# juanmc2005/diart

Measured on NVIDIA H100. Metric: audio-seconds/sec (real-time factor) at 5s/0.5s step, batch 256, higher is better.
Workload: dtype f32

## Files before the change

### diart_b200/_lib.py

```python
from __future__ import annotations

import ctypes as C
import os
from typing import Dict, Optional

import numpy as np
import torch

_HERE = os.path.dirname(os.path.abspath(__file__))
LIB_PATH = os.path.join(_HERE, "libdiartb200.so")

_lib: Optional[C.CDLL] = None


class DgTensor(C.Structure):
    _fields_ = [("name", C.c_char_p), ("data", C.c_void_p), ("numel", C.c_int64)]


_P = C.c_void_p
SIGNATURES = {
    "dg_last_error": (C.c_char_p, []),
    "dg_version": (C.c_int, []),
    "dg_launch_count": (C.c_int64, []),
    "dg_profile_enable": (C.c_int, [C.c_int]),
    "dg_profile_report": (C.c_int, [C.c_char_p, C.c_int]),
    "dg_selftest_gemm_tc": (C.c_int, [C.c_int, C.c_int, C.c_int, C.c_int, C.c_int, C.c_int, C.POINTER(C.c_float),
                                      C.POINTER(C.c_float)]),
    "dg_selftest_gemm_tc_grid": (C.c_int, [C.c_int, C.c_int, C.c_int, C.c_int, C.c_int, C.c_int, C.POINTER(C.c_int)]),
    "dg_selftest_gemm_tc_bounds": (C.c_int, [C.c_int, C.c_int, C.c_int, C.c_int, C.POINTER(C.c_int), C.POINTER(C.c_int),
                                             C.POINTER(C.c_int)]),
    "dg_selftest_wgmma_row_shift": (C.c_int, [C.c_int, C.POINTER(C.c_uint)]),
    "dg_selftest_gemm_tc_halo": (C.c_int, [C.c_int, C.c_int, C.c_int, C.c_int, C.c_int, C.c_int, C.POINTER(C.c_int),
                                           C.POINTER(C.c_int)]),
    "dg_selftest_split_f16_host": (C.c_int, [_P, C.c_longlong, _P, _P]),
    "dg_seg_create": (C.c_int, [C.POINTER(DgTensor), C.c_int, C.c_int, C.POINTER(_P)]),
    "dg_seg_dims": (C.c_int, [_P, C.c_int, C.POINTER(C.c_int), C.POINTER(C.c_int)]),
    "dg_seg_set_powerset": (C.c_int, [_P, C.c_int, C.c_int]),
    "dg_seg_forward": (C.c_int, [_P, _P, C.c_int, C.c_int, _P, _P]),
    "dg_seg_destroy": (C.c_int, [_P]),
    "dg_emb_create": (C.c_int, [C.POINTER(DgTensor), C.c_int, C.c_int, C.c_int, C.POINTER(_P)]),
    "dg_emb_dims": (C.c_int, [_P, C.c_int, C.POINTER(C.c_int), C.POINTER(C.c_int)]),
    "dg_emb_forward": (C.c_int, [_P, _P, _P, C.c_int, C.c_int, C.c_int, C.c_int, C.c_int, C.c_float, _P, _P]),
    "dg_emb_forward_rows": (C.c_int, [_P, _P, _P, C.c_int, C.c_int, C.c_int, _P, _P]),
    "dg_emb_destroy": (C.c_int, [_P]),
    "dg_emb_debug_trunk": (C.c_int, [_P, _P, C.c_int, C.c_int, C.c_int, _P, C.c_int64, _P]),
    "dg_seg_debug_stage": (C.c_int, [_P, _P, C.c_int, C.c_int, C.c_int, C.c_int, _P, C.c_int64, _P]),
    "dg_emb_debug_stage": (C.c_int, [_P, _P, _P, C.c_int, C.c_int, C.c_int, C.c_int, C.c_int, C.c_int, _P, C.c_int64, _P]),
    "dg_selftest_sinc_filters_host": (C.c_int, [_P, _P, _P]),
    "dg_selftest_fbank_tables_host": (C.c_int, [_P, _P]),
    "dg_osp": (C.c_int, [_P, C.c_int, C.c_int, C.c_int, C.c_float, C.c_float, C.c_int, _P, _P]),
    "dg_normalize_embeddings": (C.c_int, [_P, C.c_int, C.c_int, C.c_float, _P, _P]),
    "dg_cluster_create": (C.c_int, [C.c_int, C.c_int, C.c_double, C.c_double, C.c_double, C.c_int, C.POINTER(_P)]),
    "dg_cluster_set_metric": (C.c_int, [_P, C.c_int]),
    "dg_cluster_step": (C.c_int, [_P, _P, _P, C.c_int, C.c_int, C.c_int, _P, _P, _P]),
    "dg_cluster_reset": (C.c_int, [_P]),
    "dg_cluster_get_state": (C.c_int, [_P, _P, _P, C.POINTER(C.c_int)]),
    "dg_cluster_set_state": (C.c_int, [_P, _P, _P, C.c_int]),
    "dg_cluster_destroy": (C.c_int, [_P]),
    "dg_cluster_record_len": (C.c_int, [_P]),
    "dg_cluster_export_delta": (C.c_int, [_P, _P, _P]),
    "dg_cluster_merge": (C.c_int, [_P, _P, C.c_int, C.c_int, _P, C.c_int, _P]),
    "dg_pipeline_identity_export": (C.c_int, [_P, _P, _P]),
    "dg_pipeline_identity_merge": (C.c_int, [_P, _P, C.c_int, C.c_int, _P]),
    "dg_pipeline_create": (C.c_int, [_P, _P, _P, C.c_float, C.c_float, C.c_int, C.POINTER(_P)]),
    "dg_pipeline_set_hop": (C.c_int, [_P, C.c_int]),
    "dg_pipeline_step": (C.c_int, [_P, _P, C.c_int, C.c_int, _P, _P, _P, _P, _P]),
# ... 152 lines not shown
```

### diart_b200/csrc/api.cu

```cuda
#include <math.h>
#include <stdlib.h>
#include <string.h>

#include <map>
#include <sstream>
#include <vector>

#include "host.cuh"

namespace dg {

static thread_local std::string g_err;
std::atomic<long long> g_launches{0};
thread_local int g_sm_limit = 0;
void set_error(const std::string& msg) { g_err = msg; }

struct ProfRec {
  std::string name;
  cudaEvent_t a, b;
};
static bool g_prof = false;
static std::vector<ProfRec> g_recs;
static const bool g_trace = getenv("DG_TRACE_LAUNCHES") && getenv("DG_TRACE_LAUNCHES")[0] == '1';
ProfScope::ProfScope(const char* name_, cudaStream_t st_) : on(g_prof), st(st_), a(nullptr), b(nullptr), name(name_) {
// ... 337 lines not shown
    t.pool3_tile_rows = tile_rows;
  }
  if ((rc = set_weights(t, dW))) return rc;
  *halo = gemm_tc_halo(t) ? 1 : 0;
  TcGemm ref = t;
  ref.tap_boxes = 1;
  if (folded) {
    ref.Cin = Kf;
    ref.KW = 1;
    if ((rc = set_weights(ref, dWf))) return rc;
  }
  std::vector<unsigned char> first, cur;
  *equal = 1;
  for (int run = 0; run < 3; run++) {
    DG_CUDA(cudaMemset(dF.p, 0, f32_bytes + 4));
    DG_CUDA(cudaMemset(dOh.p, 0, plane_bytes + 4));
    DG_CUDA(cudaMemset(dOl.p, 0, plane_bytes + 4));
    DG_CUDA(cudaMemset(dPart.p, 0, part_bytes + 4));
    {
      SmLimit cap(run == 1 ? 3 : 0);
      if ((rc = launch_gemm_tc(run == 2 ? ref : t, nullptr))) return rc;
    }
    DG_CUDA(cudaDeviceSynchronize());
    cur.resize(f32_bytes + 2 * plane_bytes + part_bytes);
    DG_CUDA(cudaMemcpy(cur.data(), dF.p, f32_bytes, cudaMemcpyDeviceToHost));
    DG_CUDA(cudaMemcpy(cur.data() + f32_bytes, dOh.p, plane_bytes, cudaMemcpyDeviceToHost));
    DG_CUDA(cudaMemcpy(cur.data() + f32_bytes + plane_bytes, dOl.p, plane_bytes, cudaMemcpyDeviceToHost));
    DG_CUDA(cudaMemcpy(cur.data() + f32_bytes + 2 * plane_bytes, dPart.p, part_bytes, cudaMemcpyDeviceToHost));
    if (run == 0)
      first.swap(cur);
    else if (cur != first)
      *equal = 0;
  }
  return DG_OK;
}

extern "C" int dg_selftest_gemm_tc_bounds(int M, int Cin, int N, int epi, int* outside_unchanged, int* equal, int* refused) {
  const bool planes = epi == 1;
  if (M < 1 || Cin < 64 || Cin % 64 || N < 1 || N % (planes ? 32 : 4) || epi < 0 || epi > 2 || !outside_unchanged || !equal ||
      !refused) {
    set_error("dg_selftest_gemm_tc_bounds: bad arguments");
    return DG_EINVAL;
  }
  const int npad = N <= 64 && epi == 0 ? 64 : (N + 127) / 128 * 128, esize = planes ? 2 : 4;
  const int ldc = N + 40;
  const long long rows = (long long)M + 130;
  uint32_t seed = 4242u;
  auto rnd = [&]() {
    seed = seed * 1664525u + 1013904223u;
    return ((seed >> 8) & 0xFFFF) / 65536.f - 0.5f;
  };
  std::vector<float> A((size_t)M * Cin), Wnk((size_t)N * Cin), bias(N), bsc(N), bsh(N);
  for (auto& v : A) v = 2.f * rnd();
  for (auto& v : Wnk) v = 0.25f * rnd();
  for (int n = 0; n < N; n++) {
    bias[n] = rnd();
    bsc[n] = 1.f + rnd();
    bsh[n] = rnd();
  }
  const size_t dense_bytes = (size_t)M * N * esize, wide_bytes = (size_t)rows * ldc * esize + 16;
  DevBuf dA, dAh, dAl, dB, dS, dH, dD0, dD1, dW0, dW1;
  WeightPlanes dW;
  if (upload(dA, A) || upload(dB, bias) || upload(dS, bsc) || upload(dH, bsh) || upload_split(dW, Wnk, N, npad, Cin) ||
      dAh.ensure((size_t)M * Cin * 2) || dAl.ensure((size_t)M * Cin * 2) || dD0.ensure(dense_bytes) ||
      dD1.ensure(dense_bytes) || dW0.ensure(wide_bytes) || dW1.ensure(wide_bytes))
    return DG_ECUDA;
// ... 49 lines not shown
```

### diart_b200/csrc/dg_common.cuh

```cuda
#pragma once
#include <cuda_runtime.h>
#include <stdint.h>
#include <stdio.h>

#include <atomic>
#include <string>
#include <vector>

namespace dg {

void set_error(const std::string& msg);
extern std::atomic<long long> g_launches;
extern thread_local int g_sm_limit;
inline int usable_sms() {
  int dev = 0, sms = 132;
  cudaGetDevice(&dev);
  cudaDeviceGetAttribute(&sms, cudaDevAttrMultiProcessorCount, dev);
  return (g_sm_limit > 0 && g_sm_limit < sms) ? g_sm_limit : sms;
}

#define DG_CUDA(expr)                                                                   \
  do {                                                                                  \
    cudaError_t _e = (expr);                                                            \
    if (_e != cudaSuccess) {                                                            \
// ... 92 lines not shown
  int lda, Cin, KW, dil;
  long long Mtot, M;
  const void* W_hi;
  const void* W_lo;
  float w_scale;
  int Npad, N;
  const float* bias;
  const float* bn_scale;
  const float* bn_shift;
  float* out_f32;
  void* out_hi;
  void* out_lo;
  int ldc;
  int epi;
  const char* tag;
  const int* tap_off;
  int Wp, Hp, Wop, Hop, stride2, relu;
  const void* res_hi;
  const void* res_lo;
  const float* pool_w;
  float* pool_part;
  int pool_item_rows, pool_K;
  int pool_T;
  int pool3_T, pool3_tile_rows;
  int tap_boxes;
};
inline int gemm_tc_pool3_tile_rows(int item_rows) {
  for (int t = 126; t >= 96; t -= 3)
    if (item_rows % t == 0) return t;
  return 0;
}
int launch_gemm_tc(const TcGemm& g, cudaStream_t st);
bool gemm_tc_halo(const TcGemm& g);
int selftest_wgmma_row_shift(int base_offset_mode, unsigned* ok_shifts);
int launch_split_ex(const float* x, long long rows_out, int C, int ld_in, int ld_out, int pool, int item_rows,
                    const float* sc, const float* sh, void* hi, void* lo, cudaStream_t st, const int* skip_flag = nullptr);
void split_weights_host(const float* w, int N, int Npad, int K, uint16_t* hi, uint16_t* lo, float scale = 1.f);
float weight_plane_scale(const float* w, size_t n);
uint16_t host_f32_to_h16(float f);
float host_h16_to_f32(uint16_t h);
int sinc_tc_rows_per_item(const Geom& g);
size_t sinc_tc_plane_elems(int B, const Geom& g);
void sinc_tc_pack_filters(const float* filt, uint16_t* planes );
void sinc_tc_affine_consts(const float* filt, float beta, float* cf);
int launch_sinc_prep(const float* wav, const float* mean, const float* rstd, int B, const Geom& g, void* planes_hi,
                     void* planes_lo, cudaStream_t st, const int* skip_flag = nullptr);
int launch_sinc0_tc(float gamma, const float* cf_dev, const void* w_planes, int B, const Geom& g, const void* planes_hi,
                    const void* planes_lo, float* p0, cudaStream_t st, const int* skip_flag = nullptr);
struct SincStreamGeom {
  int Ls;
  int P;
  int rows;
  size_t plane;
};
SincStreamGeom sinc_stream_geom(int B, const Geom& g, int hop);
int launch_overlap_check(const float* wav, int B, int S, int hop, int* flag, cudaStream_t st);
int launch_stream_prep(const float* wav, const float* rstd, int B, const Geom& g, int hop, void* planes_hi, void* planes_lo,
                       int* flag, cudaStream_t st);
int launch_sinc0_tc_stream(const void* w_planes, int B, const Geom& g, int hop, const void* planes_hi, const void* planes_lo,
                           float* craw, const int* flag, cudaStream_t st);
size_t sinc_pool_part_floats(int B, const Geom& g, int hop);
int launch_sinc_pool_fused(const float* craw, const float* mean, const float* rstd, const float* cf, const float* hsum, float gamma,
                           int B, const Geom& g, int hop, const float* g0, const float* b0, float* part, float* sc, float* sh,
                           void* planes_hi, void* planes_lo, const int* flag, cudaStream_t st);
size_t lstm_tc_plane_elems();
int lstm_tc_rows(int B);
// ... 161 lines not shown
```

### diart_b200/csrc/gemm_tc.cu

```cuda
#include <cuda.h>
#include <cuda_bf16.h>
#include <math.h>
#include <stdlib.h>
#include <string.h>

#include <algorithm>
#include <map>
#include <mutex>
#include <string>
#include <utility>
#include <vector>

#include "dg_common.cuh"
#include "tc_ptx.cuh"

namespace dg {

constexpr int TC_BM = 128, TC_BK = 32, TC_THREADS = 384;
constexpr int TC_SMEM_MAX = 227 * 1024;

struct TcArgs {
  long long M;
  int N;
  int m_tiles, n_tiles;
// ... 26 lines not shown

__host__ __device__ constexpr bool tc_pooling(int epi) { return epi == TC_POOL || epi == TC_MAXPOOL3; }
__host__ __device__ constexpr bool tc_box_store(int epi) { return epi == TC_BIAS_F32 || epi == TC_LEAKY_BN_SPLIT || epi == TC_LEAKY_BN_F32; }

template <int BN>
struct TcSmem {
  static constexpr int A_BYTES = TC_BM * TC_BK * 2;
  static constexpr int W_BYTES = BN * TC_BK * 2;
  static constexpr int STAGE_BYTES = 2 * A_BYTES + 2 * W_BYTES;
  static constexpr int W_STAGE_BYTES = 2 * W_BYTES;
  static constexpr int NSTAGE = BN == 128 ? 4 : 6;
  static constexpr int NSTAGE_HALO = BN == 128 ? 5 : 6;
  __host__ static int halo_bytes(int cin, int rows) { return (2 * ((cin + 31) / 32) * rows * 64 + 1023) / 1024 * 1024; }
  __host__ static int halo_op_bytes(int cin, int rows) { return 2 * halo_bytes(cin, rows) + NSTAGE_HALO * W_STAGE_BYTES; }
  static constexpr int BAR_BYTES = 256;
  static constexpr int PARAM_FLOATS = 3 * BN;
  static constexpr int CHUNK_W = 64;
  static constexpr int CHUNK_FLOATS = CHUNK_W / 32 * TC_BM * 33;
  __host__ __device__ static constexpr int extra_floats(int epi) { return epi == TC_POOL ? 128 * 4 + 4 * 2 * 8 * 32 : (epi == TC_MAXPOOL3 ? 4 * 2 * 2 * 32 : 0); }
  __host__ __device__ static constexpr int consumer_floats(int epi) { return PARAM_FLOATS + (tc_pooling(epi) ? CHUNK_FLOATS + extra_floats(epi) : 0); }
  static constexpr int ACC_LD = BN + 4;
  static constexpr int BOX_BYTES = TC_BM * 128;
  __host__ __device__ static constexpr int stage_tile_bytes(int epi) {
    return tc_pooling(epi) ? 0 : (epi == TC_CONV2D ? TC_BM * ACC_LD * 4 : TC_BM * BN * 4);
  }
  __host__ __device__ static constexpr int total(int epi, int op_bytes = NSTAGE * STAGE_BYTES) {
    return op_bytes + stage_tile_bytes(epi) + BAR_BYTES + 2 * consumer_floats(epi) * 4 + 1024;
  }
};
static_assert(TcSmem<128>::total(TC_POOL) <= TC_SMEM_MAX && TcSmem<64>::total(TC_MAXPOOL3) <= TC_SMEM_MAX &&
              TcSmem<128>::total(TC_CONV2D) <= TC_SMEM_MAX && TcSmem<64>::total(TC_CONV2D) <= TC_SMEM_MAX &&
              TcSmem<32>::total(TC_CONV2D) <= TC_SMEM_MAX && TcSmem<128>::total(TC_BIAS_F32) <= TC_SMEM_MAX,
              "gemm_tc: shared memory");

template <int BN, int EPI>
__device__ __forceinline__ void tc_stage_params(const TcArgs& a, float* params, int bar, int n0, int et) {
  named_sync(bar, 128);
  for (int i = et; i < BN; i += 128) {
    const int n = n0 + i;
    const bool ok = n < a.N;
    params[i] = (ok && a.bias) ? a.bias[n] : 0.f;
    constexpr bool has_bn = EPI != TC_BIAS_F32;
    params[BN + i] = (ok && has_bn) ? a.bn_scale[n] * (EPI == TC_CONV2D ? a.acc_scale : 1.f) : 1.f;
    params[2 * BN + i] = (ok && has_bn) ? a.bn_shift[n] : 0.f;
  }
  named_sync(bar, 128);
}

template <int BN, int EPI>
__device__ __forceinline__ void tc_box_epilogue(const TcArgs& a, const float* params, float (&acc)[2][BN / 2],
                                                uint32_t tile, int quad, int lane) {
  using S = TcSmem<BN>;
  const int r0 = 16 * quad + (lane >> 2), sw = lane >> 2, cq = lane & 3;
#pragma unroll
  for (int j = 0; j < BN / 8; j++) {
    const int col = 8 * j + 2 * cq;
    const float2 bias = *reinterpret_cast<const float2*>(params + col);
    float2 bsc = make_float2(1.f, 1.f), bsh = make_float2(0.f, 0.f);
    if (EPI != TC_BIAS_F32) {
      bsc = *reinterpret_cast<const float2*>(params + BN + col);
      bsh = *reinterpret_cast<const float2*>(params + 2 * BN + col);
    }
#pragma unroll
    for (int h = 0; h < 2; h++) {
#pragma unroll
      for (int e2 = 0; e2 < 2; e2++) {
// ... 518 lines not shown
      tc_conv2d_epilogue_tile<BN>(a, params, acc_s + et * S::ACC_LD, mt, nt * BN, quad, lane);
      named_arrive(acc_free_other, 256);
    } else {
      named_sync(acc_free, 256);
      tc_box_epilogue<BN, EPI>(a, params, acc, smem_u32(tile_s), quad, lane);
      fence_proxy_async_smem();
      named_sync(bar, 128);
      if (et == 0) {
        const int m0 = mt * TC_BM, n0 = nt * BN;
        if (EPI == TC_LEAKY_BN_SPLIT) {
#pragma unroll
          for (int b = 0; b < BN / 64; b++) {
            if (n0 + 64 * b >= a.N) break;
            tma_store_2d(&tmC0, tile_s + b * S::BOX_BYTES, n0 + 64 * b, m0);
            tma_store_2d(&tmC1, tile_s + (BN / 64 + b) * S::BOX_BYTES, n0 + 64 * b, m0);
          }
        } else {
#pragma unroll
          for (int b = 0; b < BN / 32; b++) {
            if (n0 + 32 * b >= a.N) break;
            tma_store_2d(&tmC0, tile_s + b * S::BOX_BYTES, n0 + 32 * b, m0);
          }
        }
        bulk_commit();
        bulk_wait_read_all();
      }
      __syncwarp();
      named_arrive(acc_free_other, 256);
    }
  }
  if (tc_box_store(EPI) && et == 0) bulk_wait_all();
}

static int make_map(CUtensorMap* m, const void* base, long long rows, int cols, int ld, int box_cols, int box_rows,
                    bool f32 = false) {
  EncodeTiledFn fn = encode_fn();
  if (!fn) {
    set_error("cuTensorMapEncodeTiled is not available from the driver");
    return -2;
  }
  const int esize = f32 ? 4 : 2;
  cuuint64_t dims[2] = {(cuuint64_t)cols, (cuuint64_t)rows};
  cuuint64_t strides[1] = {(cuuint64_t)ld * esize};
  cuuint32_t box[2] = {(cuuint32_t)box_cols, (cuuint32_t)box_rows};
  cuuint32_t estr[2] = {1, 1};
  CUresult r = fn(m, f32 ? CU_TENSOR_MAP_DATA_TYPE_FLOAT32 : CU_TENSOR_MAP_DATA_TYPE_BFLOAT16, 2, const_cast<void*>(base), dims,
                  strides, box, estr, CU_TENSOR_MAP_INTERLEAVE_NONE,
                  box_cols * esize == 128 ? CU_TENSOR_MAP_SWIZZLE_128B : CU_TENSOR_MAP_SWIZZLE_64B,
                  CU_TENSOR_MAP_L2_PROMOTION_L2_256B, CU_TENSOR_MAP_FLOAT_OOB_FILL_NONE);
  if (r != CUDA_SUCCESS) {
    set_error("cuTensorMapEncodeTiled failed with code " + std::to_string((int)r));
    return -2;
  }
  return 0;
}

constexpr int TC_CTR_SLOTS = 1024;
__device__ unsigned g_tc_tile_ctr[TC_CTR_SLOTS][2];

static unsigned* tile_counter(cudaStream_t st) {
  static std::mutex mu;
  static std::map<std::pair<int, cudaStream_t>, int> slot_of;
  static int used[64] = {};
  int dev = 0;
  if (cudaGetDevice(&dev) != cudaSuccess || dev < 0 || dev >= 64) {
    set_error("gemm_tc: no current CUDA device");
// ... 5 lines not shown
    auto it = slot_of.find({dev, st});
    if (it != slot_of.end()) {
      slot = it->second;
    } else {
      if (used[dev] == TC_CTR_SLOTS) {
        set_error("gemm_tc: more than " + std::to_string(TC_CTR_SLOTS) + " streams have launched GEMMs on one device");
        return nullptr;
      }
      slot = slot_of[{dev, st}] = used[dev]++;
    }
  }
  void* base = nullptr;
  if (cudaGetSymbolAddress(&base, g_tc_tile_ctr) != cudaSuccess) {
    set_error("gemm_tc: cannot address the tile counters");
    return nullptr;
  }
  return static_cast<unsigned*>(base) + 2 * slot;
}

static int tc_bn(const TcGemm& g) { return g.epi == TC_MAXPOOL3 || (g.Npad == 64 && g.epi == TC_BIAS_F32) ? 64 : 128; }
static int tc_halo_rows(const TcGemm& g) {
  return (TC_BM + (g.KW - ((g.KW * g.Cin) % 32 ? 0 : 1)) * g.dil + 7) / 8 * 8;
}
template <int BN>
static int tc_halo_smem(const TcGemm& g) { return TcSmem<BN>::total(g.epi, TcSmem<BN>::halo_op_bytes(g.Cin, tc_halo_rows(g))); }

bool gemm_tc_halo(const TcGemm& g) {
  if (g.tap_boxes || g.epi == TC_CONV2D || g.tap_off || g.KW < 2 || g.dil < 1 || g.Cin % 16 || g.Cin > 128 ||
      tc_halo_rows(g) > 256)
    return false;
  return (tc_bn(g) == 64 ? tc_halo_smem<64>(g) : tc_halo_smem<128>(g)) <= TC_SMEM_MAX;
}

static int tc_setup(const TcGemm& g, int bn, int epi, bool halo, CUtensorMap* maps, TcArgs& a) {
  const int Ktot = g.KW * g.Cin, bk = TC_BK, a_rows = halo ? tc_halo_rows(g) : TC_BM;
  if (make_map(&maps[0], g.A_hi, g.Mtot, g.Cin, g.lda, bk, a_rows) || make_map(&maps[1], g.A_lo, g.Mtot, g.Cin, g.lda, bk, a_rows) ||
      make_map(&maps[2], g.W_hi, g.Npad, Ktot, Ktot, bk, bn) || make_map(&maps[3], g.W_lo, g.Npad, Ktot, Ktot, bk, bn))
    return -2;
  memset(&maps[4], 0, 2 * sizeof(CUtensorMap));
  if (epi == TC_LEAKY_BN_SPLIT) {
    if (make_map(&maps[4], g.out_hi, g.M, g.N, g.ldc, 64, TC_BM) || make_map(&maps[5], g.out_lo, g.M, g.N, g.ldc, 64, TC_BM))
      return -2;
  } else if (tc_box_store(epi)) {
    if (make_map(&maps[4], g.out_f32, g.M, g.N, g.ldc, 32, TC_BM, true)) return -2;
  }
  a = TcArgs{};
  a.M = g.M; a.N = g.N; a.n_tiles = (g.N + bn - 1) / bn;
  a.tile_rows = epi == TC_MAXPOOL3 ? g.pool3_tile_rows : TC_BM;
  a.pool3_T = g.pool3_T;
  a.m_tiles = (int)((g.M + a.tile_rows - 1) / a.tile_rows);
  a.KW = g.KW; a.dil = g.dil; a.cin_blocks = g.Cin / bk;
  a.bias = g.bias; a.bn_scale = g.bn_scale; a.bn_shift = g.bn_shift;
  a.out_f32 = g.out_f32; a.out_hi = reinterpret_cast<__nv_bfloat16*>(g.out_hi);
  a.out_lo = reinterpret_cast<__nv_bfloat16*>(g.out_lo); a.ldc = g.ldc;
  a.acc_scale = g.w_scale > 0.f ? 1.f / g.w_scale : 1.f;
  for (int j = 0; j < 9; j++) a.tap_off[j] = j < g.KW ? (g.tap_off ? g.tap_off[j] : j * g.dil) : 0;
  a.Wp = g.Wp; a.Hp = g.Hp; a.Wop = g.Wop; a.Hop = g.Hop; a.stride2 = g.stride2; a.relu = g.relu;
  a.res_hi = reinterpret_cast<const __nv_bfloat16*>(g.res_hi);
  a.res_lo = reinterpret_cast<const __nv_bfloat16*>(g.res_lo);
  a.pool_w = g.pool_w; a.pool_part = g.pool_part; a.pool_item_rows = g.pool_item_rows; a.pool_K = g.pool_K; a.pool_T = g.pool_T;
  a.cin = g.Cin;
  if (halo) {
    a.halo_rows = a_rows;
    a.wblocks = (Ktot + bk - 1) / bk;
    a.halo_bytes = bn == 64 ? TcSmem<64>::halo_bytes(g.Cin, a_rows) : TcSmem<128>::halo_bytes(g.Cin, a_rows);
    a.op_bytes = bn == 64 ? TcSmem<64>::halo_op_bytes(g.Cin, a_rows) : TcSmem<128>::halo_op_bytes(g.Cin, a_rows);
  } else {
    a.op_bytes = bn == 128 ? TcSmem<128>::NSTAGE * TcSmem<128>::STAGE_BYTES
                           : (bn == 64 ? TcSmem<64>::NSTAGE * TcSmem<64>::STAGE_BYTES : TcSmem<32>::NSTAGE * TcSmem<32>::STAGE_BYTES);
  }
  return 0;
}

static int tc_grid(const TcArgs& a) {
  const int sms = usable_sms();
  const int tiles = a.m_tiles * a.n_tiles;
  return tiles < sms ? tiles : sms;
}

template <int BN, int EPI, bool HALO>
static int launch_tc(const TcGemm& g, cudaStream_t st) {
  using S = TcSmem<BN>;
  CUtensorMap m[6];
  TcArgs a;
  if (tc_setup(g, BN, EPI, HALO, m, a)) return -2;
  if (tc_pooling(EPI) && !(a.tile_ctr = tile_counter(st))) return -2;
  auto kern = gemm_tc_kernel<BN, EPI, HALO>;
  static bool attr_done[64] = {};
  if (first_use_on_device(attr_done))
    DG_CUDA(cudaFuncSetAttribute(kern, cudaFuncAttributeMaxDynamicSharedMemorySize, HALO ? TC_SMEM_MAX : S::total(EPI)));
  kern<<<tc_grid(a), TC_THREADS, S::total(EPI, a.op_bytes), st>>>(m[0], m[1], m[2], m[3], m[4], m[5], a);
  DG_LAUNCHED();
  return 0;
}

template <int BN, int EPI>
static int launch_tc(const TcGemm& g, cudaStream_t st) {
  return gemm_tc_halo(g) ? launch_tc<BN, EPI, true>(g, st) : launch_tc<BN, EPI, false>(g, st);
}

int launch_gemm_tc(const TcGemm& g, cudaStream_t st) {
  ProfScope _ps(g.tag ? g.tag : "gemm_tc", st);
  if (g.Cin % (gemm_tc_halo(g) ? 16 : 64) || g.lda % 8 || g.ldc % (g.epi == TC_LEAKY_BN_SPLIT ? 8 : 4) ||
      (g.Npad % 128 && g.Npad != 64 && g.Npad != 32) || g.KW < 1 || g.KW > 9) {
    set_error("gemm_tc: Cin must be a multiple of 64 (a Conv1d of 2..9 taps over at most 128 channels whose tile halo fits "
              "in shared memory, e.g. Cin 80: a multiple of 16), A pitch a multiple of 8, output pitch a multiple of 4 "
              "(8 for 16-bit planes), padded N 32, 64 or a multiple of 128, at most 9 taps");
    return -1;
  }
  if (g.epi == TC_LEAKY_BN_SPLIT && g.N % 32) {
    set_error("gemm_tc (planes): N must be a multiple of 32");
    return -1;
  }
  if (tc_box_store(g.epi)) {
    const bool planes = g.epi == TC_LEAKY_BN_SPLIT;
    const uintptr_t base = planes ? ((uintptr_t)g.out_hi | (uintptr_t)g.out_lo) : (uintptr_t)g.out_f32;
    if (!base || (planes && (!g.out_hi || !g.out_lo)) || base % 16 || g.ldc < g.N || g.M >= (1LL << 31)) {
      set_error("gemm_tc: the output needs a 16-byte aligned base, a pitch of at least N and fewer than 2^31 rows");
      return -1;
    }
  }
  if (g.epi == TC_CONV2D) {
    if (g.ldc % 32 || g.N % 32 || g.Wp < 3 || g.Hp < 3 || (!g.out_hi && !g.out_f32) || g.M >= (1LL << 31)) {
      set_error("gemm_tc (conv2d): channel counts must be multiples of 32");
      return -1;
    }
    if (g.Npad == 32) return launch_tc<32, TC_CONV2D, false>(g, st);
    if (g.Npad == 64) return launch_tc<64, TC_CONV2D, false>(g, st);
    return launch_tc<128, TC_CONV2D, false>(g, st);
  }
// ... 221 lines not shown
```

### include/diart_b200.h

```cpp
#ifndef DIART_B200_H
#define DIART_B200_H

#include <stddef.h>
#include <stdint.h>

#ifdef __cplusplus
extern "C" {
#endif

#define DG_OK 0
#define DG_EINVAL (-1)
#define DG_ECUDA (-2)
#define DG_EWEIGHT (-3)
#define DG_ENCCL (-4)

typedef struct dg_tensor {
  const char* name;
  const float* data;
  int64_t numel;
} dg_tensor;

typedef struct dg_seg dg_seg;
typedef struct dg_emb dg_emb;
typedef struct dg_cluster dg_cluster;
// ... 166 lines not shown
                     double* dist_dev , void* stream);
int dg_multi_set_gallery(dg_multi* h, dg_gallery* g, double threshold);
int dg_multi_set_slot_gallery(dg_multi* h, int slot, dg_gallery* g, double threshold);
int dg_multi_set_names(dg_multi* h, int slot, uint32_t named, const int32_t* claimed_host );
int dg_multi_last_names(const dg_multi* h, int32_t* out_host , int cap, int* n);
int dg_multi_last_windows(const dg_multi* h, float* wav_dev, int n_rows);
int dg_selftest_multi_frames_host(int slots, int max_wps, int out_chunk, int out_step, int n_rates, const int32_t* rates,
                                  int n_ops, const int32_t* ops, int32_t* result, int64_t* records, int cap, int* n_records);
int dg_selftest_multi_staging_host(int slots, int C, int n_ops, const int32_t* ops, const float* samples_host, int32_t* result,
                                   float* rings_host);
int dg_selftest_gallery_plan_host(int n, const int32_t* slots, int n_keys, const int32_t* G, const double* thr,
                                  int32_t* groups_out, int32_t* segs_out, int32_t* work_out, int cap, int32_t* counts);
int dg_selftest_multi_gallery_host(int slots, int D, int M, int n_gal, const int32_t* gal, int n_ops, const double* ops,
                                   int32_t* result, char* messages, int msg_cap);
int dg_multi_create_vad(dg_seg* seg, int chunk_samples, int step_samples, int max_streams, int max_windows_per_stream,
                        double tau, int num_windows, const double* hamming_host, dg_multi** out);

typedef struct dg_resample dg_resample;
int dg_resample_create(int orig_rate, int new_rate, const float* taps_host, int width, int device, dg_resample** out);
int64_t dg_resample_out_len(const dg_resample* h, int64_t num_samples);
int dg_resample_forward(dg_resample* h, const float* in_dev, int B, int64_t L, float* out_dev, void* stream);
int dg_resample_destroy(dg_resample* h);
int dg_stream_create_resampled(int chunk_samples, int step_samples, dg_resample* rs, int max_windows, int device,
                               dg_stream** out);
int dg_stream_crop_host(dg_stream* h, int n, const int64_t* ranges_host, float* out_host);

int64_t dg_launch_count(void);
int dg_profile_enable(int enable);
int dg_selftest_gemm_tc(int M, int Cin, int KW, int dil, int N, int epi, float* max_abs_diff, float* out_rms);
int dg_selftest_gemm_tc_grid(int M, int Cin, int KW, int dil, int N, int epi, int* equal);
int dg_selftest_gemm_tc_bounds(int M, int Cin, int N, int epi, int* outside_unchanged, int* equal, int* refused);
int dg_selftest_wgmma_row_shift(int base_offset_mode, unsigned* ok_shifts);
int dg_selftest_gemm_tc_halo(int M, int Cin, int KW, int dil, int N, int epi, int* equal, int* halo);
int dg_selftest_split_f16_host(const float* x, long long n, unsigned short* hi, unsigned short* lo);
int dg_selftest_sinc_filters_host(const float* low_hz, const float* band_hz, float* filters);
int dg_selftest_fbank_tables_host(float* frame_operator, float* mel_banks);
int dg_profile_report(char* buf, int cap);

int dg_cluster_record_len(const dg_cluster* h);
int dg_cluster_export_delta(dg_cluster* h, double* record_dev, void* stream);
int dg_cluster_merge(dg_cluster* h, const double* records_dev , int world, int rank,
                     int32_t* maps_dev , int n_maps, void* stream);
int dg_pipeline_identity_export(dg_pipeline* h, double* record_dev, void* stream);
int dg_pipeline_identity_merge(dg_pipeline* h, const double* records_dev, int world, int rank, void* stream);

#ifdef __cplusplus
}
#endif
#endif
```

Before: 22460.

## Add 256-row persistent WGMMA GEMM tile path sharing weight loads across consumers

New measurement: 22700, median of 6. 1.1% higher.

```diff
diff --git a/diart_b200/_lib.py b/diart_b200/_lib.py
--- a/diart_b200/_lib.py
+++ b/diart_b200/_lib.py
@@ -32,6 +32,10 @@
     "dg_selftest_wgmma_row_shift": (C.c_int, [C.c_int, C.POINTER(C.c_uint)]),
     "dg_selftest_gemm_tc_halo": (C.c_int, [C.c_int, C.c_int, C.c_int, C.c_int, C.c_int, C.c_int, C.POINTER(C.c_int),
                                            C.POINTER(C.c_int)]),
+    "dg_selftest_gemm_tc_m256": (C.c_int, [C.c_int, C.c_int, C.c_int, C.c_int, C.c_int, C.c_int, C.POINTER(C.c_int),
+                                            C.POINTER(C.c_int)]),
+    "dg_selftest_gemm_tc_time": (C.c_int, [C.c_int, C.c_int, C.c_int, C.c_int, C.c_int, C.c_int, C.c_int, C.c_int, C.c_int,
+                                            C.POINTER(C.c_float), C.POINTER(C.c_int)]),
     "dg_selftest_split_f16_host": (C.c_int, [_P, C.c_longlong, _P, _P]),
     "dg_seg_create": (C.c_int, [C.POINTER(DgTensor), C.c_int, C.c_int, C.POINTER(_P)]),
     "dg_seg_dims": (C.c_int, [_P, C.c_int, C.POINTER(C.c_int), C.POINTER(C.c_int)]),
diff --git a/diart_b200/csrc/api.cu b/diart_b200/csrc/api.cu
--- a/diart_b200/csrc/api.cu
+++ b/diart_b200/csrc/api.cu
@@ -393,6 +393,146 @@
     else if (cur != first)
       *equal = 0;
   }
+  return DG_OK;
+}
+
+extern "C" int dg_selftest_gemm_tc_m256(int M, int Cin, int KW, int dil, int N, int epi, int* equal, int* m256) {
+  if (M < 1 || Cin < 64 || Cin % 64 || KW < 1 || KW > 9 || dil < 1 || N < 1 || N % 4 || epi < 0 || epi > 2 || (epi == 1 && N % 32) ||
+      !equal || !m256) {
+    set_error("dg_selftest_gemm_tc_m256: bad arguments");
+    return DG_EINVAL;
+  }
+  const int K = KW * Cin, npad = (N + 127) / 128 * 128;
+  uint32_t seed = 2561u;
+  auto rnd = [&]() {
+    seed = seed * 1664525u + 1013904223u;
+    return ((seed >> 8) & 0xFFFF) / 65536.f - 0.5f;
+  };
+  std::vector<float> A((size_t)M * Cin), Wnk((size_t)N * K), bias(N), bsc(N), bsh(N);
+  for (auto& v : A) v = 2.f * rnd();
+  for (auto& v : Wnk) v = 0.25f * rnd();
+  for (int n = 0; n < N; n++) {
+    bias[n] = rnd();
+    bsc[n] = 1.f + rnd();
+    bsh[n] = rnd();
+  }
+  const size_t f32_bytes = epi == 1 ? 0 : (size_t)M * N * 4, plane_bytes = epi == 1 ? (size_t)M * N * 2 : 0;
+  DevBuf dA, dAh, dAl, dB, dS, dH, dF, dOh, dOl;
+  WeightPlanes dW;
+  if (upload(dA, A) || upload(dB, bias) || upload(dS, bsc) || upload(dH, bsh) || upload_split(dW, Wnk, N, npad, K))
+    return DG_ECUDA;
+  if (dAh.ensure((size_t)M * Cin * 2) || dAl.ensure((size_t)M * Cin * 2) || dF.ensure(f32_bytes + 4) ||
+      dOh.ensure(plane_bytes + 4) || dOl.ensure(plane_bytes + 4))
+    return DG_ECUDA;
+  int rc;
+  if ((rc = launch_split_ex(dA.as<float>(), M, Cin, Cin, Cin, 0, 1, nullptr, nullptr, dAh.p, dAl.p, nullptr))) return rc;
+  TcGemm t{};
+  t.A_hi = dAh.p; t.A_lo = dAl.p; t.lda = Cin; t.Cin = Cin; t.KW = KW; t.dil = dil; t.Mtot = M; t.M = M;
+  t.N = N; t.bias = dB.as<float>(); t.bn_scale = dS.as<float>(); t.bn_shift = dH.as<float>(); t.ldc = N;
+  t.epi = epi; t.tag = "selftest_tc_m256";
+  t.out_f32 = f32_bytes ? dF.as<float>() : nullptr;
+  t.out_hi = plane_bytes ? dOh.p : nullptr;
+  t.out_lo = plane_bytes ? dOl.p : nullptr;
+  if ((rc = set_weights(t, dW))) return rc;
+  {
+    SmLimit cap(3);
+    *m256 = gemm_tc_m256(t) ? 1 : 0;
+  }
+  TcGemm ref = t;
+  ref.tap_boxes = 1;
+  std::vector<unsigned char> first, cur;
+  *equal = 1;
+  for (int run = 0; run < 3; run++) {
+    DG_CUDA(cudaMemset(dF.p, 0, f32_bytes + 4));
+    DG_CUDA(cudaMemset(dOh.p, 0, plane_bytes + 4));
+    DG_CUDA(cudaMemset(dOl.p, 0, plane_bytes + 4));
+    {
+      SmLimit cap(run == 0 ? 3 : 7);
+      if ((rc = launch_gemm_tc(run == 2 ? ref : t, nullptr))) return rc;
+    }
+    DG_CUDA(cudaDeviceSynchronize());
+    cur.resize(f32_bytes + 2 * plane_bytes);
+    DG_CUDA(cudaMemcpy(cur.data(), dF.p, f32_bytes, cudaMemcpyDeviceToHost));
+    DG_CUDA(cudaMemcpy(cur.data() + f32_bytes, dOh.p, plane_bytes, cudaMemcpyDeviceToHost));
+    DG_CUDA(cudaMemcpy(cur.data() + f32_bytes + plane_bytes, dOl.p, plane_bytes, cudaMemcpyDeviceToHost));
+    if (run == 0)
+      first.swap(cur);
+    else if (cur != first)
+      *equal = 0;
+  }
+  return DG_OK;
+}
+
+extern "C" int dg_selftest_gemm_tc_time(int M, int Cin, int KW, int dil, int N, int epi, int item_rows, int rows128, int reps,
+                                        float* ms, int* mode) {
+  if (M < 1 || Cin < 16 || Cin % 16 || KW < 1 || KW > 9 || dil < 1 || N < 1 || N % 4 || (epi == 1 && N % 32) || epi < 0 || epi > 5 || epi == 3 ||
+      reps < 1 || !ms || !mode || ((epi == 4 || epi == 5) && (item_rows < 128 || M % item_rows)) || (epi == 5 && N > 64)) {
+    set_error("dg_selftest_gemm_tc_time: bad arguments");
+    return DG_EINVAL;
+  }
+  const int K = KW * Cin, npad = epi == 5 || N == 64 ? 64 : (N + 127) / 128 * 128, tail = 64;
+  const int tile_rows = epi == 5 ? gemm_tc_pool3_tile_rows(item_rows) : 128;
+  if (epi == 5 && !tile_rows) {
+    set_error("dg_selftest_gemm_tc_time: no MaxPool1d(3) tile for these items");
+    return DG_EINVAL;
+  }
+  const long long m_tiles = (M + tile_rows - 1) / tile_rows;
+  uint32_t seed = 31337u;
+  auto rnd = [&]() {
+    seed = seed * 1664525u + 1013904223u;
+    return ((seed >> 8) & 0xFFFF) / 65536.f - 0.5f;
+  };
+  std::vector<float> A((size_t)(M + tail) * Cin, 0.f), Wnk((size_t)N * K), bias(N), bsc(N), bsh(N), pw((size_t)M * 4);
+  for (size_t i = 0; i < (size_t)M * Cin; i++) A[i] = 2.f * rnd();
+  for (auto& v : Wnk) v = 0.25f * rnd();
+  for (int n = 0; n < N; n++) {
+    bias[n] = rnd();
+    bsc[n] = 1.f + rnd();
+    bsh[n] = rnd();
+  }
+  for (auto& v : pw) v = rnd() + 0.5f;
+  const size_t f32_bytes = epi == 5 ? (size_t)(M / 3) * N * 4 : (size_t)M * N * 4;
+  const size_t part_bytes = (size_t)m_tiles * 2 * TC_POOL_SLOTS * N * 4;
+  DevBuf dA, dAh, dAl, dB, dS, dH, dPw, dF, dOh, dOl, dPart;
+  WeightPlanes dW;
+  if (upload(dA, A) || upload(dB, bias) || upload(dS, bsc) || upload(dH, bsh) || upload(dPw, pw) || upload_split(dW, Wnk, N, npad, K) ||
+      dAh.ensure((size_t)(M + tail) * Cin * 2) || dAl.ensure((size_t)(M + tail) * Cin * 2) || dF.ensure(f32_bytes) ||
+      dOh.ensure((size_t)M * N * 2) || dOl.ensure((size_t)M * N * 2) || dPart.ensure(part_bytes))
+    return DG_ECUDA;
+  int rc;
+  if ((rc = launch_split_ex(dA.as<float>(), M + tail, Cin, Cin, Cin, 0, 1, nullptr, nullptr, dAh.p, dAl.p, nullptr))) return rc;
+  TcGemm t{};
+  t.A_hi = dAh.p; t.A_lo = dAl.p; t.lda = Cin; t.Cin = Cin; t.KW = KW; t.dil = dil; t.Mtot = M + tail; t.M = M;
+  t.N = N; t.bias = dB.as<float>(); t.bn_scale = dS.as<float>(); t.bn_shift = dH.as<float>(); t.ldc = N;
+  t.epi = epi; t.tag = "selftest_tc_time"; t.tap_boxes = rows128;
+  if (epi == 1) {
+    t.out_hi = dOh.p; t.out_lo = dOl.p;
+  } else if (epi != 4) {
+    t.out_f32 = dF.as<float>();
+  }
+  if (epi == 4) {
+    t.pool_w = dPw.as<float>(); t.pool_part = dPart.as<float>(); t.pool_item_rows = item_rows; t.pool_K = 3; t.pool_T = item_rows;
+  }
+  if (epi == 5) {
+    t.pool_part = dPart.as<float>(); t.pool_item_rows = item_rows; t.pool3_T = item_rows / 3 - 2; t.pool3_tile_rows = tile_rows;
+  }
+  if ((rc = set_weights(t, dW))) return rc;
+  *mode = gemm_tc_m256(t) ? 2 : (gemm_tc_halo(t) ? 1 : 0);
+  for (int i = 0; i < reps / 5 + 2; i++)
+    if ((rc = launch_gemm_tc(t, nullptr))) return rc;
+  cudaEvent_t e0, e1;
+  DG_CUDA(cudaEventCreate(&e0));
+  DG_CUDA(cudaEventCreate(&e1));
+  DG_CUDA(cudaEventRecord(e0, nullptr));
+  for (int i = 0; i < reps && !rc; i++) rc = launch_gemm_tc(t, nullptr);
+  DG_CUDA(cudaEventRecord(e1, nullptr));
+  DG_CUDA(cudaEventSynchronize(e1));
+  float total = 0.f;
+  cudaEventElapsedTime(&total, e0, e1);
+  cudaEventDestroy(e0);
+  cudaEventDestroy(e1);
+  if (rc) return rc;
+  *ms = total / reps;
   return DG_OK;
 }
 
diff --git a/diart_b200/csrc/dg_common.cuh b/diart_b200/csrc/dg_common.cuh
--- a/diart_b200/csrc/dg_common.cuh
+++ b/diart_b200/csrc/dg_common.cuh
@@ -148,6 +148,7 @@
 }
 int launch_gemm_tc(const TcGemm& g, cudaStream_t st);
 bool gemm_tc_halo(const TcGemm& g);
+bool gemm_tc_m256(const TcGemm& g);
 int selftest_wgmma_row_shift(int base_offset_mode, unsigned* ok_shifts);
 int launch_split_ex(const float* x, long long rows_out, int C, int ld_in, int ld_out, int pool, int item_rows,
                     const float* sc, const float* sh, void* hi, void* lo, cudaStream_t st, const int* skip_flag = nullptr);
diff --git a/diart_b200/csrc/gemm_tc.cu b/diart_b200/csrc/gemm_tc.cu
--- a/diart_b200/csrc/gemm_tc.cu
+++ b/diart_b200/csrc/gemm_tc.cu
@@ -82,6 +82,20 @@
               TcSmem<128>::total(TC_CONV2D) <= TC_SMEM_MAX && TcSmem<64>::total(TC_CONV2D) <= TC_SMEM_MAX &&
               TcSmem<32>::total(TC_CONV2D) <= TC_SMEM_MAX && TcSmem<128>::total(TC_BIAS_F32) <= TC_SMEM_MAX,
               "gemm_tc: shared memory");
+
+struct TcSmemM256 {
+  using S = TcSmem<128>;
+  static constexpr int A_BYTES = 2 * TC_BM * TC_BK * 2;
+  static constexpr int STAGE_BYTES = 2 * A_BYTES + 2 * S::W_BYTES;
+  static constexpr int NSTAGE = 3;
+  static constexpr int OP_BYTES = NSTAGE * STAGE_BYTES;
+  __host__ __device__ static constexpr int total(int epi, int nstage = NSTAGE) {
+    return nstage * STAGE_BYTES + S::stage_tile_bytes(epi) + S::BAR_BYTES + 2 * S::consumer_floats(epi) * 4 + 1024;
+  }
+};
+static_assert(TcSmemM256::STAGE_BYTES == 48 * 1024 && TcSmemM256::total(TC_LEAKY_BN_SPLIT) <= TC_SMEM_MAX &&
+              TcSmemM256::total(TC_LEAKY_BN_SPLIT, 4) > TC_SMEM_MAX && TcSmemM256::total(TC_POOL) > TC_SMEM_MAX,
+              "gemm_tc (256-row tiles): shared memory");
 
 template <int BN, int EPI>
 __device__ __forceinline__ void tc_stage_params(const TcArgs& a, float* params, int bar, int n0, int et) {
@@ -666,6 +680,208 @@
   if (tc_box_store(EPI) && et == 0) bulk_wait_all();
 }
 
+template <int EPI>
+__device__ __forceinline__ void tc_box_epilogue_half(const TcArgs& a, const float* params, float (&acc)[2][64], uint32_t buf,
+                                                     int HALF, int quad, int lane) {
+  using S = TcSmem<128>;
+  constexpr int BN = 128;
+  const int r0 = 16 * quad + (lane >> 2), sw = lane >> 2, cq = lane & 3;
+#pragma unroll
+  for (int j = 8 * HALF; j < 8 * HALF + 8; j++) {
+    const int col = 8 * j + 2 * cq;
+    const float2 bias = *reinterpret_cast<const float2*>(params + col);
+    float2 bsc = make_float2(1.f, 1.f), bsh = make_float2(0.f, 0.f);
+    if (EPI != TC_BIAS_F32) {
+      bsc = *reinterpret_cast<const float2*>(params + BN + col);
+      bsh = *reinterpret_cast<const float2*>(params + 2 * BN + col);
+    }
+#pragma unroll
+    for (int h = 0; h < 2; h++) {
+#pragma unroll
+      for (int e2 = 0; e2 < 2; e2++) {
+        const int row = 64 * h + r0 + 8 * e2;
+        float x0 = fmaf(acc[h][4 * j + 2 * e2], a.acc_scale, bias.x);
+        float x1 = fmaf(acc[h][4 * j + 2 * e2 + 1], a.acc_scale, bias.y);
+        if (EPI != TC_BIAS_F32) {
+          x0 = fmaf(leaky(x0), bsc.x, bsh.x);
+          x1 = fmaf(leaky(x1), bsc.y, bsh.y);
+        }
+        if (EPI == TC_LEAKY_BN_SPLIT) {
+          uint16_t h0, l0, h1, l1;
+          split_h16(x0, h0, l0);
+          split_h16(x1, h1, l1);
+          const int off = row * 128 + (((j & 7) ^ sw) << 4) + 4 * cq;
+          st_shared_u32(buf + off, pack_u16x2(h0, h1));
+          st_shared_u32(buf + S::BOX_BYTES + off, pack_u16x2(l0, l1));
+        } else {
+          const int q = 2 * (j & 3) + (cq >> 1);
+          const int off = (j / 4 - 2 * HALF) * S::BOX_BYTES + row * 128 + ((q ^ sw) << 4) + 8 * (cq & 1);
+          st_shared_v2(buf + off, x0, x1);
+        }
+      }
+    }
+  }
+}
+
+template <int EPI>
+__global__ void __launch_bounds__(TC_THREADS, 1)
+gemm_tc_m256_kernel(const __grid_constant__ CUtensorMap tmA_hi, const __grid_constant__ CUtensorMap tmA_lo,
+                    const __grid_constant__ CUtensorMap tmW_hi, const __grid_constant__ CUtensorMap tmW_lo,
+                    const __grid_constant__ CUtensorMap tmC0, const __grid_constant__ CUtensorMap tmC1, TcArgs a) {
+  constexpr int BN = 128;
+  using S = TcSmem<BN>;
+  using S2 = TcSmemM256;
+  static_assert(tc_box_store(EPI), "gemm_tc_m256_kernel: box epilogues only");
+  constexpr int NSTAGE = S2::NSTAGE;
+  extern __shared__ unsigned char smem_raw[];
+  unsigned char* smem = reinterpret_cast<unsigned char*>((reinterpret_cast<uintptr_t>(smem_raw) + 1023) & ~uintptr_t(1023));
+  unsigned char* tile_s = smem + S2::OP_BYTES;
+  uint64_t* bars = reinterpret_cast<uint64_t*>(tile_s + S::stage_tile_bytes(EPI));
+  uint64_t* full = bars;
+  uint64_t* empty = bars + NSTAGE;
+  uint64_t* tile_full = bars + 2 * NSTAGE;
+  uint64_t* tile_empty = tile_full + 2;
+  volatile int* tile_idx = reinterpret_cast<volatile int*>(tile_empty + 2);
+  float* cons = reinterpret_cast<float*>(reinterpret_cast<unsigned char*>(bars) + S::BAR_BYTES);
+
+  const int warp = __shfl_sync(0xffffffffu, (int)(threadIdx.x >> 5), 0), lane = threadIdx.x & 31;
+  const int wg = warp >> 2;
+  const int m256_tiles = (a.m_tiles + 1) >> 1, num_tiles = m256_tiles * a.n_tiles;
+  const int kblocks = a.KW * a.cin_blocks;
+
+  if (threadIdx.x == 0) {
+    for (int s = 0; s < NSTAGE; s++) {
+      mbar_init(&full[s], 1);
+      mbar_init(&empty[s], 2);
+    }
+    for (int i = 0; i < 2; i++) {
+      mbar_init(&tile_full[i], 1);
+      mbar_init(&tile_empty[i], 256);
+    }
+    asm volatile("fence.mbarrier_init.release.cluster;" ::: "memory");
+  }
+  __syncthreads();
+
+  if (wg == 0) {
+    setmaxnreg_dec<40>();
+    if (threadIdx.x == 0) {
+      int stage = 0, phase = 0;
+      for (int i = 0, tile = blockIdx.x;; i++) {
+        const int s = i & 1;
+        mbar_wait(&tile_empty[s], ((i >> 1) & 1) ^ 1);
+        if (tile >= num_tiles) {
+          tile_idx[s] = -1;
+          mbar_arrive(&tile_full[s]);
+          break;
+        }
+        tile_idx[s] = tile;
+        mbar_arrive(&tile_full[s]);
+        const int mt = tile / a.n_tiles, nt = tile - mt * a.n_tiles;
+        const int m0 = mt * 2 * TC_BM, n0 = nt * BN;
+        for (int j = 0; j < a.KW; j++) {
+          for (int cb = 0; cb < a.cin_blocks; cb++) {
+            mbar_wait(&empty[stage], phase ^ 1);
+            unsigned char* st = smem + stage * S2::STAGE_BYTES;
+            mbar_expect_tx(&full[stage], S2::STAGE_BYTES);
+            const int kcol = (j * a.cin_blocks + cb) * TC_BK;
+            tma_load_2d(st, &tmA_hi, cb * TC_BK, m0 + a.tap_off[j], &full[stage]);
+            tma_load_2d(st + S2::A_BYTES, &tmA_lo, cb * TC_BK, m0 + a.tap_off[j], &full[stage]);
+            tma_load_2d(st + 2 * S2::A_BYTES, &tmW_hi, kcol, n0, &full[stage]);
+            tma_load_2d(st + 2 * S2::A_BYTES + S::W_BYTES, &tmW_lo, kcol, n0, &full[stage]);
+            if (++stage == NSTAGE) {
+              stage = 0;
+              phase ^= 1;
+            }
+          }
+        }
+        tile = (int)gridDim.x + (int)atomicAdd(&a.tile_ctr[0], 1u);
+      }
+      __threadfence();
+      if (atomicAdd(&a.tile_ctr[1], 1u) == gridDim.x - 1) {
+        atomicExch(&a.tile_ctr[0], 0u);
+        atomicExch(&a.tile_ctr[1], 0u);
+      }
+    }
+    return;
+  }
+  setmaxnreg_inc<232>();
+  const int c = wg - 1, quad = warp & 3, et = threadIdx.x - 128 * wg;
+  float* params = cons + c * S::consumer_floats(EPI);
+  const int bar = 1 + c;
+  for (int n = 0;; n++) {
+    mbar_wait(&tile_full[n & 1], (n >> 1) & 1);
+    const int tile = tile_idx[n & 1];
+    mbar_arrive(&tile_empty[n & 1]);
+    if (tile < 0) break;
+    const int mt2 = tile / a.n_tiles, nt = tile - mt2 * a.n_tiles;
+    if (a.n_tiles > 1 || n == 0) tc_stage_params<BN, EPI>(a, params, bar, nt * BN, et);
+    const int pos = n * kblocks;
+    int stage = pos % NSTAGE, phase = (pos / NSTAGE) & 1;
+    float acc[2][BN / 2];
+#pragma unroll
+    for (int i = 0; i < BN / 2; i++) acc[0][i] = acc[1][i] = 0.f;
+    for (int kb = 0; kb < kblocks; kb++) {
+      mbar_wait(&full[stage], phase);
+      const uint32_t st = smem_u32(smem + stage * S2::STAGE_BYTES), sa = st + (uint32_t)c * (TC_BM * TC_BK * 2);
+      const uint32_t sw = st + 2 * S2::A_BYTES;
+      const uint64_t w_hi = wg_desc_sw64(sw), w_lo = wg_desc_sw64(sw + S::W_BYTES);
+      constexpr uint64_t HALF = (uint64_t)((64 * TC_BK * 2) >> 4);
+      wg_fence_acc(acc[0]);
+      wg_fence_acc(acc[1]);
+      wg_fence();
+#pragma unroll
+      for (int ks = 0; ks < TC_BK / 16; ks++) {
+        const uint64_t adv = (uint64_t)((ks * 32) >> 4);
+        const uint64_t a_hi = wg_desc_sw64(sa) + adv, a_lo = wg_desc_sw64(sa + S2::A_BYTES) + adv;
+#pragma unroll
+        for (int h = 0; h < 2; h++) {
+          wgmma_ss<BN>(acc[h], a_lo + h * HALF, w_hi + adv, (kb | ks) != 0);
+          wgmma_ss<BN>(acc[h], a_hi + h * HALF, w_lo + adv, 1);
+          wgmma_ss<BN>(acc[h], a_hi + h * HALF, w_hi + adv, 1);
+        }
+      }
+      wg_commit();
+      wg_wait<1>();
+      wg_fence_acc(acc[0]);
+      wg_fence_acc(acc[1]);
+      if (kb > 0 && et == 0) mbar_arrive(&empty[stage == 0 ? NSTAGE - 1 : stage - 1]);
+      if (++stage == NSTAGE) {
+        stage = 0;
+        phase ^= 1;
+      }
+    }
+    wg_wait<0>();
+    wg_fence_acc(acc[0]);
+    wg_fence_acc(acc[1]);
+    if (et == 0) mbar_arrive(&empty[stage == 0 ? NSTAGE - 1 : stage - 1]);
+    const int mt = 2 * mt2 + c;
+    const bool rows = mt < a.m_tiles;
+    if (rows) {
+      const int m0 = mt * TC_BM, n0 = nt * BN;
+      unsigned char* buf = tile_s + c * 2 * S::BOX_BYTES;
+#pragma unroll
+      for (int H = 0; H < 2; H++) {
+        if (et == 0) bulk_wait_read_all();
+        named_sync(bar, 128);
+        tc_box_epilogue_half<EPI>(a, params, acc, smem_u32(buf), H, quad, lane);
+        fence_proxy_async_smem();
+        named_sync(bar, 128);
+        if (et == 0 && n0 + 64 * H < a.N) {
+          if (EPI == TC_LEAKY_BN_SPLIT) {
+            tma_store_2d(&tmC0, buf, n0 + 64 * H, m0);
+            tma_store_2d(&tmC1, buf + S::BOX_BYTES, n0 + 64 * H, m0);
+          } else {
+            tma_store_2d(&tmC0, buf, n0 + 64 * H, m0);
+            if (n0 + 64 * H + 32 < a.N) tma_store_2d(&tmC0, buf + S::BOX_BYTES, n0 + 64 * H + 32, m0);
+          }
+          bulk_commit();
+        }
+      }
+    }
+  }
+  if (et == 0) bulk_wait_all();
+}
+
 static int make_map(CUtensorMap* m, const void* base, long long rows, int cols, int ld, int box_cols, int box_rows,
                     bool f32 = false) {
   EncodeTiledFn fn = encode_fn();
@@ -737,8 +953,13 @@
   return (tc_bn(g) == 64 ? tc_halo_smem<64>(g) : tc_halo_smem<128>(g)) <= TC_SMEM_MAX;
 }
 
-static int tc_setup(const TcGemm& g, int bn, int epi, bool halo, CUtensorMap* maps, TcArgs& a) {
-  const int Ktot = g.KW * g.Cin, bk = TC_BK, a_rows = halo ? tc_halo_rows(g) : TC_BM;
+bool gemm_tc_m256(const TcGemm& g) {
+  if (g.tap_boxes || gemm_tc_halo(g) || tc_bn(g) != 128 || !tc_box_store(g.epi) || g.KW * g.Cin < 1536) return false;
+  return (g.M + 2 * TC_BM - 1) / (2 * TC_BM) * ((g.N + 127) / 128) >= usable_sms();
+}
+
+static int tc_setup(const TcGemm& g, int bn, int epi, bool halo, CUtensorMap* maps, TcArgs& a, bool m256 = false) {
+  const int Ktot = g.KW * g.Cin, bk = TC_BK, a_rows = halo ? tc_halo_rows(g) : (m256 ? 2 * TC_BM : TC_BM);
   if (make_map(&maps[0], g.A_hi, g.Mtot, g.Cin, g.lda, bk, a_rows) || make_map(&maps[1], g.A_lo, g.Mtot, g.Cin, g.lda, bk, a_rows) ||
       make_map(&maps[2], g.W_hi, g.Npad, Ktot, Ktot, bk, bn) || make_map(&maps[3], g.W_lo, g.Npad, Ktot, Ktot, bk, bn))
     return -2;
@@ -770,6 +991,8 @@
     a.wblocks = (Ktot + bk - 1) / bk;
     a.halo_bytes = bn == 64 ? TcSmem<64>::halo_bytes(g.Cin, a_rows) : TcSmem<128>::halo_bytes(g.Cin, a_rows);
     a.op_bytes = bn == 64 ? TcSmem<64>::halo_op_bytes(g.Cin, a_rows) : TcSmem<128>::halo_op_bytes(g.Cin, a_rows);
+  } else if (m256) {
+    a.op_bytes = TcSmemM256::OP_BYTES;
   } else {
     a.op_bytes = bn == 128 ? TcSmem<128>::NSTAGE * TcSmem<128>::STAGE_BYTES
                            : (bn == 64 ? TcSmem<64>::NSTAGE * TcSmem<64>::STAGE_BYTES : TcSmem<32>::NSTAGE * TcSmem<32>::STAGE_BYTES);
@@ -799,8 +1022,25 @@
   return 0;
 }
 
+template <int EPI>
+static int launch_tc_m256(const TcGemm& g, cudaStream_t st) {
+  CUtensorMap m[6];
+  TcArgs a;
+  if (tc_setup(g, 128, EPI, false, m, a, true) || !(a.tile_ctr = tile_counter(st))) return -2;
+  auto kern = gemm_tc_m256_kernel<EPI>;
+  static bool attr_done[64] = {};
+  if (first_use_on_device(attr_done))
+    DG_CUDA(cudaFuncSetAttribute(kern, cudaFuncAttributeMaxDynamicSharedMemorySize, TcSmemM256::total(EPI)));
+  const int tiles = (a.m_tiles + 1) / 2 * a.n_tiles, sms = usable_sms();
+  kern<<<tiles < sms ? tiles : sms, TC_THREADS, TcSmemM256::total(EPI), st>>>(m[0], m[1], m[2], m[3], m[4], m[5], a);
+  DG_LAUNCHED();
+  return 0;
+}
+
 template <int BN, int EPI>
 static int launch_tc(const TcGemm& g, cudaStream_t st) {
+  if constexpr (BN == 128 && tc_box_store(EPI))
+    if (gemm_tc_m256(g)) return launch_tc_m256<EPI>(g, st);
   return gemm_tc_halo(g) ? launch_tc<BN, EPI, true>(g, st) : launch_tc<BN, EPI, false>(g, st);
 }
 
diff --git a/include/diart_b200.h b/include/diart_b200.h
--- a/include/diart_b200.h
+++ b/include/diart_b200.h
@@ -222,6 +222,9 @@
 int dg_selftest_gemm_tc_bounds(int M, int Cin, int N, int epi, int* outside_unchanged, int* equal, int* refused);
 int dg_selftest_wgmma_row_shift(int base_offset_mode, unsigned* ok_shifts);
 int dg_selftest_gemm_tc_halo(int M, int Cin, int KW, int dil, int N, int epi, int* equal, int* halo);
+int dg_selftest_gemm_tc_m256(int M, int Cin, int KW, int dil, int N, int epi, int* equal, int* m256);
+int dg_selftest_gemm_tc_time(int M, int Cin, int KW, int dil, int N, int epi, int item_rows, int rows128, int reps, float* ms,
+                             int* mode);
 int dg_selftest_split_f16_host(const float* x, long long n, unsigned short* hi, unsigned short* lo);
 int dg_selftest_sinc_filters_host(const float* low_hz, const float* band_hz, float* filters);
 int dg_selftest_fbank_tables_host(float* frame_operator, float* mel_banks);
```
